# zhanwenchen/pbe

Hardware: AMD Instinct MI355X
Metric: 512x512 images/sec @50 PLMS steps scale=5 (higher is better)
Workload: dtype fp16; 1 GPU; BASELINE configs[1]: batch=4/GPU, 512x512, 50 PLMS steps (51 U-Net calls at batch 8), scale=5, fp16 activations + fp32 accumulate, name-seeded random-init U-Net + VAE + CLIP ViT-L/14 weights; the context-independent prefix of each guidance pair (first ResBlock + first self-attention) is evaluated once; per_gpu_batch=4, global_batch=4, plms_steps=50, parallelism=batch-sharded x1, no per-step collective

## Files before the change

### pbe_amd/csrc/igemm_kernel.h

```cpp
#pragma once
#include <cstddef>
#include <type_traits>
#include <utility>
#include "common.h"
#include "../../include/pbe_hip.h"

struct IGemmP {
    const h16* A; const h16* A2; const h16* W;
    long lda, lda2, ldw;
    long sA, sW;
    int M, N, K, K1;
    int splits;
    int m_fast;
    int tdiv; unsigned mg_tdiv;
    int split_per;
    int sv_ns;
    int sv_gdiv; unsigned mg_sv_gdiv;
    int H, Wd, C1, C2, Ho, Wo, cstride, pad, ups, cb;
    int phase;
    int th;
    int hw; unsigned mg_hw, mg_wo;
    int per_blk; unsigned mg_per_blk, mg_kb;
    int h_hw2, h_hps, h_nsub, h_rows, h_tpi; unsigned mg_h_tpi, mh_hps, mh_hw2; int h_lgw, h_lgimg;
    h16* C;
// ... 130 lines not shown
                    const float v = 8 * c + 4 * q + e < len ? (float)x[4 * q + e] * al : 0.f;
                    word |= mx8_e4m3(v * inv) << (8 * e);
                }
                w[2 * cc + q] = (int)word;
            }
        }
        *reinterpret_cast<i32x4_*>(dst + 16 * hf) = w;
    }
    return se;
}

__device__ __forceinline__ int mx8_range(const IGemmP& p, int n) {
    int r = -1;
    for (int q = 0; q < p.mx_nr; ++q)
        if (p.mx_c0[q] <= n && (r < 0 || p.mx_c0[q] > p.mx_c0[r])) r = q;
    return r;
}

__device__ __forceinline__ void mx8_vt_scale(const IGemmP& p, int r, int b, int c, int tok, int se) {
    const int D = p.mx_D, DV = p.mx_DV;
    const int h = c / D, d = c - h * D;
    unsigned char* sp = p.mx_scale[r] + (((long)b * p.mx_H + h) * (p.mx_N >> 5) + (tok >> 5)) * DV;
    sp[d] = (unsigned char)se;
    if (d == D - 1)
        for (int q = D; q < DV; q += 8) *reinterpret_cast<unsigned long long*>(sp + q) = 0x7f7f7f7f7f7f7f7full;
}

__device__ __forceinline__ void mx8_vt_block(const IGemmP& p, int r, const h16* src, int b, int c, int tok) {
    const int se = mx8_block_lds(src, 32, p.mx_alpha[r], p.mx_data[r] + ((long)b * p.mx_H * p.mx_D + c) * p.mx_N + tok);
    mx8_vt_scale(p, r, b, c, tok, se);
}

__device__ __forceinline__ void mx8_vt_block_pair(const IGemmP& p, int r, const h16* src, int b, int c, int tok, int hf) {
    typedef int i32x4_ __attribute__((ext_vector_type(4)));
    const float al = p.mx_alpha[r];
    const h16x8 x[2] = {*reinterpret_cast<const h16x8*>(src + 16 * hf), *reinterpret_cast<const h16x8*>(src + 16 * hf + 8)};
    float amax = 0.f;
#pragma unroll
    for (int c2 = 0; c2 < 2; ++c2)
#pragma unroll
        for (int e = 0; e < 8; ++e) amax = fmaxf(amax, fabsf((float)x[c2][e] * al));
    amax = fmaxf(amax, __shfl_xor(amax, 32, 64));
    const int se = mx8_scale_exp(amax);
    const float inv = __uint_as_float((unsigned)(254 - se) << 23);
    i32x4_ w;
#pragma unroll
    for (int q = 0; q < 4; ++q) {
        unsigned word = 0;
#pragma unroll
        for (int e = 0; e < 4; ++e) word |= mx8_e4m3((float)x[q >> 1][4 * (q & 1) + e] * al * inv) << (8 * e);
        w[q] = (int)word;
    }
    *reinterpret_cast<i32x4_*>(p.mx_data[r] + ((long)b * p.mx_H * p.mx_D + c) * p.mx_N + tok + 16 * hf) = w;
    if (hf == 0) mx8_vt_scale(p, r, b, c, tok, se);
}

__device__ __forceinline__ void mx8_token_blocks(const IGemmP& p, int r, const h16* st, int ld, int rows, int x0, int cols, int mrow0, int t0, int nt) {
    const int D = p.mx_D, Hh = p.mx_H, Nt = p.mx_N, DP = p.mx_DP;
    const int nbh = (D + 31) >> 5, npb = DP >> 5;
    auto nblk = [&](int x) { const int hh = x / D; return hh * nbh + (x - hh * D + 31) / 32; };
    const int c0 = p.mx_c0[r], rel0 = x0 - c0, rel1 = min(x0 + cols, c0 + Hh * D) - c0;
    if (rel1 <= rel0) return;
    const int b0 = nblk(rel0), cnt = nblk(rel1) - b0;
    const float al = p.mx_alpha[r];
    for (int idx = t0; idx < rows * cnt; idx += nt) {
        const int row = idx / cnt, gb = b0 + (idx - row * cnt);
        const int m = mrow0 + row;
        if (m >= p.M) continue;
        const int h = gb / nbh, j = gb - h * nbh, len = min(32, D - 32 * j);
        unsigned char* dst = p.mx_data[r] + (long)m * Hh * DP + h * DP + 32 * j;
        const int se = mx8_block_lds(st + row * ld + (c0 + h * D + 32 * j - x0), len, al, dst);
        const int b = m / Nt, n = m - b * Nt;
        unsigned char* sp = p.mx_scale[r] + (((long)b * Hh + h) * npb + j) * Nt + n;
        sp[0] = (unsigned char)se;
        if (j == nbh - 1 && npb > nbh) {
            typedef int i32x4_ __attribute__((ext_vector_type(4)));
            *reinterpret_cast<i32x4_*>(dst + 32) = (i32x4_){0, 0, 0, 0};
            *reinterpret_cast<i32x4_*>(dst + 48) = (i32x4_){0, 0, 0, 0};
            sp[Nt] = 127;
        }
    }
}

template <int BM, int BN, int NWM, int NWN, int MODE, int S, int HPA = 0, bool PP = false, bool F8 = false, int EX = 0>
#ifndef PBE_EX_MINWAVES
#define PBE_EX_MINWAVES 2
#endif
__global__ void __launch_bounds__(NWM* NWN * 64, ((EX & 4) != 0 && NWM * NWN == 4 && S == 2) ? PBE_EX_MINWAVES : 1) igemm_kernel(const IGemmP p) {
    constexpr bool EXL = (EX & 1) != 0, EXS = (EX & 2) != 0, EXV = (EX & 4) != 0, EXM = (EX & EX_MX) != 0;
    constexpr int EXF = EX & 7;
    constexpr int NW = NWM * NWN, NT = NW * 64;
    constexpr int D = S - 1;
    constexpr int WM = BM / NWM, WN = BN / NWN, TM = WM / 16, TN = WN / 16;
    constexpr int A_BYTES = BM * 128, W_BYTES = BN * 128, STAGE = A_BYTES + W_BYTES;
    constexpr int PA = BM / 8, PW = BN / 8;
    constexpr int LA = PA / NW, LW = (PW + NW - 1) / NW, LPT = LA + LW;
    constexpr int CLD = BN + 8;
    constexpr int RING = MODE == 2 ? 2 * HPA * 128 + S * W_BYTES : S * STAGE;
    static_assert(S >= 2 && S <= 4 && PA % NW == 0 && BM % 16 == 0 && BN % 16 == 0, "A pieces must divide over the waves (weight pieces may be padded)");
    static_assert(MODE != 2 || (HPA % 8 == 0 && HPA >= BM), "halo image must hold the tile");
    static_assert(EXF == 0 || (MODE == 0 && !F8), "extended epilogue: dense fp16 tiles only");
    static_assert(!EXM || (MODE == 0 && !EXS && (F8 || EXF == (EX_LN | EX_VT))), "MX-fp8 copy-out: the fp8 tiles and the q|k|v^T form");
    extern __shared__ __attribute__((aligned(16))) unsigned char smem[];

    const int tid = threadIdx.x, lane = tid & 63;
    const int wave = __builtin_amdgcn_readfirstlane(tid >> 6);
    const int wm = wave % NWM, wn = wave / NWM;
    PBE_ACC_DECL;
#if PBE_PRIO_MODE == 2
    if (NW == 8 && __builtin_amdgcn_readfirstlane(wave) >= 4) __builtin_amdgcn_s_setprio(1);
#endif
    PBE_STAMP(0);
    PBE_STAMP(7);
    int tile;
    {
        const int nwg = gridDim.x, id = blockIdx.x, q = nwg >> 3, r = nwg & 7, xcd = id & 7;
        tile = (xcd < r ? xcd * (q + 1) : r * (q + 1) + (xcd - r) * q) + (id >> 3);
    }
    const int tq = (int)udiv_mg((unsigned)tile, (unsigned)p.tdiv, p.mg_tdiv), tr = tile - tq * p.tdiv;
    const int tn_i = p.m_fast ? tq : tr, tm_i = p.m_fast ? tr : tq;
    const int m0 = tm_i * BM, n0 = tn_i * BN;
    const long bz = blockIdx.y;
#ifdef PBE_STAMPS
    if (m0 >= 0) PBE_STAMP(14);
#endif

    const int lrow = lane >> 3;
    const int gch = (lane & 7) ^ lrow;
    const h16* zsrc = reinterpret_cast<const h16*>(g_pbe_zero16);

    const h16* a_cur[LA];
    const h16* a_alt[LA];
#pragma unroll
    for (int i = 0; i < LA; ++i) {
        const int m = min(m0 + (wave * LA + i) * 8 + lrow, p.M - 1);
        a_cur[i] = p.A + bz * p.sA + (long)m * p.lda + gch * 8;
        a_alt[i] = p.A2 ? p.A2 + (long)m * p.lda2 + gch * 8 - p.K1 : a_cur[i];
    }
    int* tab = reinterpret_cast<int*>(smem + RING);
    float* svec = reinterpret_cast<float*>(smem + (RING > WM * CLD * 2 ? RING : WM * CLD * 2) + (MODE == 1 ? 9 * BM * 4 : 0));
    const int sv_ns = p.sv_ns;
    if (MODE == 1) {
        const int hw = p.hw, Hv = p.H << p.ups, Wv = p.Wd << p.ups;
        const int py = p.phase ? (int)(blockIdx.y >> 1) : 0, px = p.phase ? (int)(blockIdx.y & 1) : 0;
        for (int row = tid; row < BM; row += NT) {
            const int m = m0 + row;
            const bool rok = m < p.M;
            const int b = (int)udiv_mg((unsigned)m, (unsigned)hw, p.mg_hw), rem = m - b * hw;
            const int oy = (int)udiv_mg((unsigned)rem, (unsigned)p.Wo, p.mg_wo), ox = rem - oy * p.Wo;
            const int iy0 = oy * p.cstride - p.pad, ix0 = ox * p.cstride - p.pad;
            if (p.phase) {
#pragma unroll
                for (int tp = 0; tp < 4; ++tp) {
                    const int iy = oy - 1 + py + (tp >> 1), ix = ox - 1 + px + (tp & 1);
                    const bool ok = rok && (unsigned)iy < (unsigned)p.H && (unsigned)ix < (unsigned)p.Wd;
                    tab[tp * BM + row] = ok ? (b * p.H + iy) * p.Wd + ix : -1;
                }
                continue;
            }
#pragma unroll
            for (int tp = 0; tp < 9; ++tp) {
                const int iy = iy0 + tp / 3, ix = ix0 + tp % 3;
                const bool ok = rok && (unsigned)iy < (unsigned)Hv && (unsigned)ix < (unsigned)Wv;
                tab[tp * BM + row] = ok ? (b * p.H + (iy >> p.ups)) * p.Wd + (ix >> p.ups) : -1;
            }
        }
// ... 541 lines not shown
            const int nl = wn * WN + i * 16 + fq * 4;
            const int n = n0 + nl;
            float ali = al, c1a[4] = {0.f, 0.f, 0.f, 0.f};
            if constexpr (EXV) ali = (p.alpha_cols > 0 && n >= p.alpha_cols) ? 1.f : al;
            if constexpr (EXL) {
                if (EXF != 7 || p.ln_stat) {
                    const f32x4 c1 = *reinterpret_cast<const f32x4*>(lnc + nl);
#pragma unroll
                    for (int r = 0; r < 4; ++r) c1a[r] = ali * c1[r];
                }
            }
            float bn[4] = {0.f, 0.f, 0.f, 0.f};
            if (F) {
                const f32x4 t = *reinterpret_cast<const f32x4*>(svec + nl);
#pragma unroll
                for (int r = 0; r < 4; ++r) bn[r] = t[r];
            } else if (!p.sv_ok && p.bias && !p.bias_row) {
#pragma unroll
                for (int r = 0; r < 4; ++r) bn[r] = (n + r < p.N) ? p.bias[n + r] : 0.f;
            }
#pragma unroll
            for (int j = 0; j < TM; ++j) {
                const int ml = (ONE_PASS ? wm * WM : 0) + j * 16 + fr;
                float v[4];
                float add[4] = {bn[0], bn[1], bn[2], bn[3]};
                if (!F) {
                    const int m = m0 + g * GR + ml;
                    if (p.sv_ok) {
                        const f32x4 t = *reinterpret_cast<const f32x4*>(svec + (sv_ns > 1 ? (g * GR + ml) / p.group_rows : 0) * BN + nl);
#pragma unroll
                        for (int r = 0; r < 4; ++r) add[r] = t[r];
                    } else if (p.rowvec && m < p.M) {
                        const h16* rv = p.rowvec + (long)(m / p.group_rows) * p.ldv + n;
#pragma unroll
                        for (int r = 0; r < 4; ++r)
                            if (n + r < p.N) add[r] = bn[r] + (float)rv[r];
                    }
                }
                if constexpr (F8) {
                    const float sm = sca[g * GR + ml] * al;
                    const f32x4 sn = *reinterpret_cast<const f32x4*>(scw + nl);
#pragma unroll
                    for (int r = 0; r < 4; ++r) v[r] = __builtin_fmaf(acc[i][j][r], sm * sn[r], add[r]);
                } else if constexpr (EXF != 0) {
                    if constexpr (EXL && EXF != 7) {
                        const float ars = ali * ln_rs[j];
#pragma unroll
                        for (int r = 0; r < 4; ++r) v[r] = __builtin_fmaf(acc[i][j][r], ars, __builtin_fmaf(ln_nm[j], c1a[r], add[r]));
                    } else {
                        const float ars = (EXL && p.ln_stat) ? ali * ln_rs[j] : ali, nmj = (EXL && p.ln_stat) ? ln_nm[j] : 0.f;
#pragma unroll
                        for (int r = 0; r < 4; ++r) v[r] = __builtin_fmaf(acc[i][j][r], ars, __builtin_fmaf(nmj, c1a[r], add[r]));
                    }
                    if constexpr (VT) {
#pragma unroll
                        for (int r = 0; r < 4; ++r) sC[(nl + r) * CLDT + ml] = (h16)v[r];
                        continue;
                    }
                } else {
#pragma unroll
                    for (int r = 0; r < 4; ++r) v[r] = __builtin_fmaf(acc[i][j][r], al, add[r]);
                }
                if (!F) {
                    const int m = m0 + g * GR + ml;
                    if (p.bias && p.bias_row) {
                        const float bm = (m < p.M) ? p.bias[m] : 0.f;
#pragma unroll
                        for (int r = 0; r < 4; ++r) v[r] += bm;
                    }
                }
                if (A == PBE_ACT_GEGLU) {
                    h16x2 o2 = {(h16)(v[0] * gelu_erf_f(v[1])), (h16)(v[2] * gelu_erf_f(v[3]))};
                    *reinterpret_cast<h16x2*>(sC + ml * CLD + (nl >> 1)) = o2;
                } else {
                    apply_act4(v, A);
                    h16x4 o;
#pragma unroll
                    for (int r = 0; r < 4; ++r) o[r] = (h16)v[r];
                    *reinterpret_cast<h16x4*>(sC + ml * CLD + nl) = o;
                }
            }
        }
    };
    auto copy_out = [&](int g, auto GG) {
        constexpr bool gg = decltype(GG)::value;
        constexpr int cpr = gg ? CPR / 2 : CPR;
        constexpr int TOT = GR * cpr, IT = (TOT + NT - 1) / NT;
        constexpr int UB = !ONE_PASS ? (IT % 2 == 0 ? 2 : 1) : (IT % 5 == 0 ? 5 : (IT % 4 == 0 ? 4 : (IT % 3 == 0 ? 3 : (IT % 2 == 0 ? 2 : 1))));
        const int Nout = gg ? p.N >> 1 : p.N, nb = gg ? n0 >> 1 : n0;
        if constexpr (EXM && !gg) {
            if (p.mx_crow) {
                constexpr int BPR = BN / 32;
                for (int idx = tid; idx < GR * BPR; idx += NT) {
                    const int row = idx / BPR, cb = idx - row * BPR;
                    const int m = m0 + g * GR + row, n = n0 + cb * 32;
                    if (m >= p.M || n >= p.N) continue;
                    mx8_vt_block(p, 0, sC + row * CLD + cb * 32, (int)bz, m, n);
                }
                return;
            }
            const int r = mx8_range(p, n0);
            if (r < 0) return;
            if (p.mx_layout[r] == PBE_MX8_VT) {
                if constexpr (EXV) {
                    constexpr int BPR = GR / 32;
                    for (int idx = tid; idx < BN * BPR; idx += NT) {
                        const int crow = idx / BPR, tb = idx - crow * BPR;
                        const int m = m0 + tb * 32;
                        if (m >= p.M || n0 + crow >= p.N) continue;
                        const int b = m / p.mx_N;
                        mx8_vt_block(p, r, sC + crow * CLDT + tb * 32, b, n0 - p.mx_c0[r] + crow, m - b * p.mx_N);
                    }
                }
                return;
            }
            mx8_token_blocks(p, r, sC, CLD, GR, n0, BN, m0 + g * GR, tid, NT);
            return;
        }
        if constexpr (EXV && !gg) {
            if (vtile) {
                constexpr int tpr = GR / 8;
                for (int idx = tid; idx < BN * tpr; idx += NT) {
                    const int crow = idx / tpr, tch = idx - crow * tpr;
                    const int m = m0 + tch * 8, c = n0 - p.vt_col0 + crow;
                    if (m >= p.M || n0 + crow >= p.N) continue;
                    const int b = m / p.vt_tok, tok = m - b * p.vt_tok;
                    *reinterpret_cast<h16x8*>(p.vt + (long)b * p.vt_bs + (long)c * p.vt_rs + tok) = *reinterpret_cast<const h16x8*>(sC + crow * CLDT + tch * 8);
                }
                return;
            }
        }
        if constexpr (EXS && !gg) {
            if (p.rstat) {
                constexpr int RPP = NT / 8, CPL = (CPR + 7) / 8, NIT = (GR + RPP - 1) / RPP;
                const int l8 = tid & 7, rr = tid >> 3;
                h16x8 r[NIT][CPL];
                if (Rb) {
#pragma unroll
                    for (int it = 0; it < NIT; ++it) {
                        const int row = it * RPP + rr, m = m0 + g * GR + row;
#pragma unroll
                        for (int c = 0; c < CPL; ++c) {
                            const int ch = l8 + 8 * c, n = n0 + ch * 8;
                            if (row < GR && m < p.M && ch < CPR && n < p.N) r[it][c] = *reinterpret_cast<const h16x8*>(Rb + (long)m * p.ldr + n);
                        }
                    }
                }
#pragma unroll
                for (int it = 0; it < NIT; ++it) {
                    const int row = it * RPP + rr, m = m0 + g * GR + row;
                    const bool rok = row < GR && m < p.M;
                    float s1 = 0.f, s2 = 0.f;
#pragma unroll
                    for (int c = 0; c < CPL; ++c) {
                        const int ch = l8 + 8 * c, n = n0 + ch * 8;
                        if (!(rok && ch < CPR && n < p.N)) continue;
                        h16x8 v = *reinterpret_cast<const h16x8*>(sC + row * CLD + ch * 8);
                        if (Rb) {
#pragma unroll
                            for (int e = 0; e < 8; ++e) v[e] = (h16)((float)v[e] + (float)r[it][c][e]);
                        }
#pragma unroll
                        for (int e = 0; e < 8; ++e) { const float f = (float)v[e]; s1 += f; s2 = __builtin_fmaf(f, f, s2); }
                        *reinterpret_cast<h16x8*>(Cb + (long)m * p.ldc + n) = v;
                    }
#pragma unroll
                    for (int o = 1; o < 8; o <<= 1) { s1 += __shfl_xor(s1, o, 64); s2 += __shfl_xor(s2, o, 64); }
                    if (rok && l8 == 0) *reinterpret_cast<float2*>(p.rstat + 2 * ((long)tn_i * p.rstat_ld + m)) = make_float2(s1, s2);
                }
                return;
            }
        }
        if constexpr (GS_OK && !gg) {
            if (p.gstat) {
                constexpr int RSL = NT / CPR, GB = 4;
                float* red = reinterpret_cast<float*>(smem + GS_OFF);
                const int slot = tid / CPR, ch = tid - slot * CPR, n = n0 + ch * 8;
                float ca[8], cq[8];
#pragma unroll
                for (int e = 0; e < 8; ++e) { ca[e] = 0.f; cq[e] = 0.f; }
                if (slot < RSL && n < p.N) {
                    for (int r0 = slot; r0 < GR; r0 += RSL * GB) {
                        h16x8 v[GB], r[GB];
                        bool ok[GB];
#pragma unroll
                        for (int u = 0; u < GB; ++u) {
                            const int row = r0 + u * RSL, m = m0 + row;
                            ok[u] = row < GR && m < p.M;
                            if (ok[u] && Rb) r[u] = *reinterpret_cast<const h16x8*>(Rb + (long)m * p.ldr + n);
                        }
#pragma unroll
                        for (int u = 0; u < GB; ++u)
                            if (ok[u]) v[u] = *reinterpret_cast<const h16x8*>(sC + (r0 + u * RSL) * CLD + ch * 8);
#pragma unroll
                        for (int u = 0; u < GB; ++u) {
                            if (!ok[u]) continue;
                            if (Rb) {
#pragma unroll
                                for (int e = 0; e < 8; ++e) v[u][e] = (h16)((float)v[u][e] + (float)r[u][e]);
                            }
#pragma unroll
                            for (int e = 0; e < 8; ++e) { const float f = (float)v[u][e]; ca[e] += f; cq[e] = __builtin_fmaf(f, f, cq[e]); }
                            *reinterpret_cast<h16x8*>(Cb + out_row(m0 + r0 + u * RSL) * p.ldc + n) = v[u];
                        }
                    }
                }
                if (slot < RSL) {
#pragma unroll
                    for (int e = 0; e < 8; ++e) *reinterpret_cast<float2*>(red + ((slot * BN) + ch * 8 + e) * 2) = make_float2(ca[e], cq[e]);
                }
                __syncthreads();
                float* col = red + RSL * BN * 2;
                if (tid < BN) {
                    float a = 0.f, q = 0.f;
                    for (int sl = 0; sl < RSL; ++sl) { const float2 t = *reinterpret_cast<const float2*>(red + (sl * BN + tid) * 2); a += t.x; q += t.y; }
                    *reinterpret_cast<float2*>(col + tid * 2) = make_float2(a, q);
                }
                __syncthreads();
                const int cg = p.gs_cg, gl = tid;
                if (gl * cg < BN && n0 + gl * cg < p.N) {
                    float a = 0.f, q = 0.f;
                    for (int c = gl * cg; c < (gl + 1) * cg; ++c) { const float2 t = *reinterpret_cast<const float2*>(col + c * 2); a += t.x; q += t.y; }
                    const int b = m0 / p.gs_hw, blk = (m0 - b * p.gs_hw) / BM, nblk = p.gs_hw / BM;
                    *reinterpret_cast<float2*>(p.gstat + (((long)b * nblk + blk) * p.gs_groups + n0 / cg + gl) * 2) = make_float2(a, q);
                }
                return;
            }
        }
        if (p.vec) {
            for (int it0 = 0; it0 < IT; it0 += UB) {
                h16x8 v[UB], r[UB];
                long go[UB];
                int lo[UB];
#pragma unroll
                for (int u = 0; u < UB; ++u) {
                    const int idx = tid + (it0 + u) * NT;
                    const int row = idx / cpr, ch = idx - row * cpr;
                    const int m = m0 + g * GR + row, n = nb + ch * 8;
                    const bool ok = idx < TOT && m < p.M && n < Nout;
                    go[u] = ok ? out_row(m) * p.ldc + n : -1;
                    lo[u] = row * CLD + ch * 8;
                    if (ok && Rb) r[u] = *reinterpret_cast<const h16x8*>(Rb + (long)m * p.ldr + n);
                }
#pragma unroll
                for (int u = 0; u < UB; ++u)
                    if (go[u] >= 0) v[u] = *reinterpret_cast<const h16x8*>(sC + lo[u]);
#pragma unroll
                for (int u = 0; u < UB; ++u) {
                    if (go[u] < 0) continue;
                    if (Rb) {
#pragma unroll
                        for (int e = 0; e < 8; ++e) v[u][e] = (h16)((float)v[u][e] + (float)r[u][e]);
                    }
                    *reinterpret_cast<h16x8*>(Cb + go[u]) = v[u];
                }
            }
            return;
        }
        for (int idx = tid; idx < TOT; idx += NT) {
            const int row = idx / cpr, ch = idx - row * cpr;
            const int m = m0 + g * GR + row, n = nb + ch * 8;
            if (m >= p.M || n >= Nout) continue;
            const h16x8 v = *reinterpret_cast<const h16x8*>(sC + row * CLD + ch * 8);
#pragma unroll
            for (int e = 0; e < 8; ++e) {
                if (n + e < Nout) {
                    float f = (float)v[e];
                    if (Rb) f += (float)Rb[(long)m * p.ldr + n + e];
                    Cb[out_row(m) * p.ldc + n + e] = (h16)f;
                }
            }
        }
    };
    const bool fast = p.sv_ok && sv_ns == 1 && !(p.bias && p.bias_row);
#pragma unroll 1
    for (int g = 0; g < NG; ++g) {
        __syncthreads();
        if (ONE_PASS || wm == g) {
            auto run = [&](auto FAST) {
                if constexpr (EXV) {
                    if (vtile) { stage(g, FAST, std::integral_constant<int, 0>{}, std::true_type{}); return; }
                }
                if constexpr (ARMS) {
                    switch (p.act) {
                        case 1: stage(g, FAST, std::integral_constant<int, 1>{}, std::false_type{}); break;
                        case 2: stage(g, FAST, std::integral_constant<int, 2>{}, std::false_type{}); break;
                        case 3: stage(g, FAST, std::integral_constant<int, 3>{}, std::false_type{}); break;
                        case PBE_ACT_GEGLU: stage(g, FAST, std::integral_constant<int, PBE_ACT_GEGLU>{}, std::false_type{}); break;
                        default: stage(g, FAST, std::integral_constant<int, 0>{}, std::false_type{}); break;
                    }
                } else {
                    stage(g, FAST, std::integral_constant<int, -1>{}, std::false_type{});
                }
            };
            if (fast) run(std::true_type{});
            else run(std::false_type{});
        }
        __syncthreads();
#ifdef PBE_STAMPS
        if (g == NG - 1) PBE_STAMP(5);
#endif
        if (p.act == PBE_ACT_GEGLU) copy_out(g, std::true_type{});
        else copy_out(g, std::false_type{});
    }
    PBE_STAMP(6);
    PBE_STAMP(8);
}

static __global__ void __launch_bounds__(256) splitk_reduce_kernel(const IGemmP p) {
    const long i = (long)blockIdx.x * 256 + threadIdx.x;
    const int n4 = p.N >> 2;
    if (i >= (long)p.M * n4) return;
    const int m = (int)(i / n4), n = (int)(i - (long)m * n4) * 4;
    float ev[4] = {0.f, 0.f, 0.f, 0.f}, rs[4] = {0.f, 0.f, 0.f, 0.f};
    if (p.bias) {
#pragma unroll
        for (int r = 0; r < 4; ++r) ev[r] = p.bias_row ? p.bias[m] : p.bias[n + r];
    }
    if (p.rowvec) {
        const h16* rv = p.rowvec + (long)(m / p.group_rows) * p.ldv + n;
#pragma unroll
        for (int r = 0; r < 4; ++r) ev[r] += (float)rv[r];
    }
    if (p.resid && p.act != PBE_ACT_GEGLU) {
#pragma unroll
        for (int r = 0; r < 4; ++r) rs[r] = (float)p.resid[(long)m * p.ldr + n + r];
    }
    const float* sl = p.ws + (long)m * p.N + n;
    const long zs = (long)p.M * p.N;
    f32x4 a = {0.f, 0.f, 0.f, 0.f};
    int z = 0;
    for (; z + 4 <= p.splits; z += 4) {
        const f32x4 t0 = *reinterpret_cast<const f32x4*>(sl + (z + 0) * zs), t1 = *reinterpret_cast<const f32x4*>(sl + (z + 1) * zs);
        const f32x4 t2 = *reinterpret_cast<const f32x4*>(sl + (z + 2) * zs), t3 = *reinterpret_cast<const f32x4*>(sl + (z + 3) * zs);
        a += t0; a += t1; a += t2; a += t3;
    }
    for (; z < p.splits; ++z) a += *reinterpret_cast<const f32x4*>(sl + z * zs);
    float v[4];
#pragma unroll
    for (int r = 0; r < 4; ++r) v[r] = a[r] * p.alpha + ev[r];
    if (p.act == PBE_ACT_GEGLU) {
        h16x2 o2 = {(h16)(v[0] * gelu_erf_f(v[1])), (h16)(v[2] * gelu_erf_f(v[3]))};
        *reinterpret_cast<h16x2*>(p.C + (long)m * p.ldc + (n >> 1)) = o2;
        return;
    }
    h16x4 o;
#pragma unroll
    for (int r = 0; r < 4; ++r) {
        const float f = (float)(h16)apply_act(v[r], p.act) + rs[r];
        o[r] = (h16)f;
    }
    *reinterpret_cast<h16x4*>(p.C + (long)m * p.ldc + n) = o;
}

static inline bool al16(const void* p) { return (reinterpret_cast<uintptr_t>(p) & 15) == 0; }
struct Plan { int cfg; int splits; };
enum : unsigned {
    F_DENSE = 1u << 0,
    F_CONV = 1u << 1,
    F_HALO = 1u << 2,
    F_EX = 1u << 3,
    F_F8 = 1u << 4,
    F_ASTAT = 1u << 5,
    F_FORCED = 1u << 6,
};
struct TileCfg { int bm, bn, nwm, nwn, s, slots_per_cu; double eff, eff_shallow; int hpa; unsigned forms; int f8; };
static constexpr TileCfg kTiles[] = {
    {256, 256, 2, 4, 2, 1, 1.00, 0.82, 0, F_DENSE | F_CONV, 3},
    {256, 128, 4, 2, 3, 1, 0.82, 0.72, 0, F_DENSE | F_CONV, 3},
    {128, 256, 2, 4, 3, 1, 0.75, 0.66, 0, F_DENSE | F_CONV, 3},
    {128, 128, 2, 2, 2, 2, 0.88, 1.00, 0, F_DENSE | F_CONV | F_EX | F_F8, 3},
    {128, 64, 2, 2, 2, 3, 0.65, 0.84, 0, F_DENSE | F_CONV | F_EX | F_F8, 4},
    {64, 128, 2, 2, 2, 3, 0.65, 0.85, 0, F_DENSE | F_CONV | F_EX, 6},
    {64, 64, 2, 2, 2, 4, 0.60, 0.80, 0, F_DENSE | F_CONV | F_EX | F_F8, 6},
    {256, 320, 2, 4, 2, 1, 1.05, 0.80, 0, F_DENSE | F_CONV, 8},
    {128, 320, 2, 4, 2, 1, 0.96, 0.95, 0, F_DENSE | F_CONV | F_EX | F_F8, 8},
    {128, 160, 2, 2, 2, 2, 0.90, 0.97, 0, F_DENSE | F_CONV | F_EX | F_F8, 9},
    {256, 160, 4, 2, 3, 1, 1.40, 1.40, 392, F_HALO, 9},
    {128, 160, 4, 2, 3, 1, 1.20, 1.20, 264, F_HALO, 9},
    {128, 320, 2, 4, 2, 1, 1.25, 1.25, 264, F_HALO, 9},
    {256, 128, 4, 2, 3, 1, 1.30, 1.30, 392, F_HALO, 9},
// ... 246 lines not shown
```

### pbe_amd/csrc/norm.hip

```cpp
#include "common.h"
#include "../../include/pbe_hip.h"

#define GN_MAX_C 4096
#define GN_MAX_CHUNKS 256

__device__ __forceinline__ const h16* gn_src(const h16* X, const h16* X2, int C1, int C2, long row, int v) {
    const int c = v * 8;
    return (c < C1) ? X + row * C1 + c : X2 + row * C2 + (c - C1);
}

__global__ void __launch_bounds__(256) gn_stats_kernel(const h16* X, const h16* X2, float* part, int HW, int C1, int C2,
                                                        int groups, int rows_per_block, int TX, int TY) {
    __shared__ float s_sum[GN_MAX_C], s_sq[GN_MAX_C];
    __shared__ float s_pa[256 * 8], s_pq[256 * 8];
    const int C = C1 + C2, C8 = C >> 3, cg = C / groups;
    const int tid = threadIdx.x, tx = tid % TX, ty = tid / TX;
    const int b = blockIdx.y, chunk = blockIdx.x;
    const int r0 = chunk * rows_per_block;
    const int r1 = min(HW, r0 + rows_per_block);
    if (ty < TY) {
        for (int v = tx; v < C8; v += TX) {
            float a[8], q[8];
#pragma unroll
            for (int e = 0; e < 8; ++e) { a[e] = 0.f; q[e] = 0.f; }
            int r = r0 + ty;
            for (; r + 3 * TY < r1; r += 4 * TY) {
                h16x8 x[4];
#pragma unroll
                for (int u = 0; u < 4; ++u) x[u] = *reinterpret_cast<const h16x8*>(gn_src(X, X2, C1, C2, (long)b * HW + r + u * TY, v));
#pragma unroll
                for (int u = 0; u < 4; ++u)
#pragma unroll
                    for (int e = 0; e < 8; ++e) { const float f = (float)x[u][e]; a[e] += f; q[e] += f * f; }
            }
            for (; r < r1; r += TY) {
                const h16x8 x = *reinterpret_cast<const h16x8*>(gn_src(X, X2, C1, C2, (long)b * HW + r, v));
#pragma unroll
                for (int e = 0; e < 8; ++e) { const float f = (float)x[e]; a[e] += f; q[e] += f * f; }
            }
            if (TY == 1) {
#pragma unroll
                for (int e = 0; e < 8; ++e) { s_sum[v * 8 + e] = a[e]; s_sq[v * 8 + e] = q[e]; }
            } else {
#pragma unroll
                for (int e = 0; e < 8; ++e) { s_pa[tid * 8 + e] = a[e]; s_pq[tid * 8 + e] = q[e]; }
            }
        }
    }
    __syncthreads();
    if (TY > 1) {
        for (int c = tid; c < C; c += 256) {
            const int v = c >> 3, e = c & 7;
            float a = 0.f, q = 0.f;
            for (int y = 0; y < TY; ++y) { a += s_pa[(y * TX + v) * 8 + e]; q += s_pq[(y * TX + v) * 8 + e]; }
            s_sum[c] = a; s_sq[c] = q;
        }
        __syncthreads();
    }
    if (tid < groups) {
        float a = 0.f, q = 0.f;
        for (int c = tid * cg; c < (tid + 1) * cg; ++c) { a += s_sum[c]; q += s_sq[c]; }
        float* dst = part + (((long)b * gridDim.x + chunk) * groups + tid) * 2;
        dst[0] = a; dst[1] = q;
    }
}

__global__ void __launch_bounds__(256) gn_apply_kernel(const h16* X, const h16* X2, const float* part, const float* gamma,
                                                        const float* beta, h16* Y, int HW, int C1, int C2, int groups,
                                                        int nchunks, int rows_per_block, int TX, int TY, float eps, int silu) {
    __shared__ float s_mean[64], s_rstd[64];
    __shared__ double s_a[256], s_q[256];
    const int C = C1 + C2, C8 = C >> 3, cg = C / groups;
    const int tid = threadIdx.x, tx = tid % TX, ty = tid / TX;
    const int b = blockIdx.y;
    {
        const int slices = 256 / groups;
        const int g = tid % groups, sl = tid / groups;
        double a = 0.0, q = 0.0;
        if (sl < slices)
            for (int c = sl; c < nchunks; c += slices) {
                const float* src = part + (((long)b * nchunks + c) * groups + g) * 2;
                a += (double)src[0]; q += (double)src[1];
            }
        s_a[tid] = a; s_q[tid] = q;
        __syncthreads();
        if (tid < groups) {
            double ta = 0.0, tq = 0.0;
            for (int s = 0; s < slices; ++s) { ta += s_a[s * groups + tid]; tq += s_q[s * groups + tid]; }
            const double n = (double)HW * cg;
            const double mean = ta / n;
            double var = tq / n - mean * mean;
            if (var < 0.0) var = 0.0;
            s_mean[tid] = (float)mean;
            s_rstd[tid] = (float)(1.0 / sqrt(var + (double)eps));
        }
        __syncthreads();
    }
    const int r0 = blockIdx.x * rows_per_block;
    const int r1 = min(HW, r0 + rows_per_block);
    if (ty >= TY) return;
    for (int v = tx; v < C8; v += TX) {
        float sc[8], sh[8];
#pragma unroll
        for (int e = 0; e < 8; ++e) {
            const int c = v * 8 + e, g = c / cg;
            const float a = s_rstd[g] * gamma[c];
            sc[e] = a; sh[e] = beta[c] - s_mean[g] * a;
        }
        int r = r0 + ty;
        for (; r + 3 * TY < r1; r += 4 * TY) {
            h16x8 x[4];
#pragma unroll
            for (int u = 0; u < 4; ++u) x[u] = *reinterpret_cast<const h16x8*>(gn_src(X, X2, C1, C2, (long)b * HW + r + u * TY, v));
#pragma unroll
            for (int u = 0; u < 4; ++u) {
                h16x8 y;
#pragma unroll
                for (int e = 0; e < 8; ++e) {
                    float f = (float)x[u][e] * sc[e] + sh[e];
                    if (silu) f = silu_f(f);
                    y[e] = (h16)f;
                }
                *reinterpret_cast<h16x8*>(Y + ((long)b * HW + r + u * TY) * C + v * 8) = y;
            }
        }
        for (; r < r1; r += TY) {
            const long row = (long)b * HW + r;
            const h16x8 x = *reinterpret_cast<const h16x8*>(gn_src(X, X2, C1, C2, row, v));
            h16x8 y;
#pragma unroll
            for (int e = 0; e < 8; ++e) {
                float f = (float)x[e] * sc[e] + sh[e];
                if (silu) f = silu_f(f);
                y[e] = (h16)f;
            }
            *reinterpret_cast<h16x8*>(Y + row * C + v * 8) = y;
        }
    }
}

#define GN_SMALL_ROWS 12
__global__ void __launch_bounds__(256) gn_small_kernel(const h16* X, const h16* X2, const float* gamma, const float* beta, h16* Y,
                                                        int HW, int C1, int C2, int groups, float eps, int silu) {
    __shared__ float s_a[4], s_q[4];
    const int C = C1 + C2, cg = C / groups, TX = cg >> 3, TY = 256 / TX;
    const int tid = threadIdx.x, lane = tid & 63, wave = tid >> 6;
    const int tx = tid % TX, ty = tid / TX;
    const int g = blockIdx.x, b = blockIdx.y;
    const int v = (g * cg >> 3) + tx;
    const bool act = ty < TY;
    h16x8 x[GN_SMALL_ROWS];
    float a = 0.f, q = 0.f;
#pragma unroll
    for (int u = 0; u < GN_SMALL_ROWS; ++u) {
        const int r = ty + u * TY;
        if (act && r < HW) {
            x[u] = *reinterpret_cast<const h16x8*>(gn_src(X, X2, C1, C2, (long)b * HW + r, v));
#pragma unroll
            for (int e = 0; e < 8; ++e) { const float f = (float)x[u][e]; a += f; q += f * f; }
        }
    }
    a = wave_sum(a); q = wave_sum(q);
    if (lane == 0) { s_a[wave] = a; s_q[wave] = q; }
    __syncthreads();
    const double n = (double)HW * cg;
    const double mean = ((double)s_a[0] + s_a[1] + s_a[2] + s_a[3]) / n;
    double var = ((double)s_q[0] + s_q[1] + s_q[2] + s_q[3]) / n - mean * mean;
    if (var < 0.0) var = 0.0;
    const float mu = (float)mean, rstd = (float)(1.0 / sqrt(var + (double)eps));
    if (!act) return;
    float sc[8], sh[8];
#pragma unroll
    for (int e = 0; e < 8; ++e) {
        const int c = v * 8 + e;
        sc[e] = rstd * gamma[c];
        sh[e] = beta[c] - mu * sc[e];
    }
#pragma unroll
    for (int u = 0; u < GN_SMALL_ROWS; ++u) {
        const int r = ty + u * TY;
        if (r < HW) {
            h16x8 y;
#pragma unroll
            for (int e = 0; e < 8; ++e) {
                float f = (float)x[u][e] * sc[e] + sh[e];
                if (silu) f = silu_f(f);
                y[e] = (h16)f;
            }
            *reinterpret_cast<h16x8*>(Y + ((long)b * HW + r) * C + v * 8) = y;
        }
    }
}

int g_pbe_gn_rows = 16;
int g_pbe_gn_apply2_rows = 8;
int g_pbe_gn_apply_rows = 4;
static void gn_geometry(int HW, int C, int* nchunks, int* rpb, int* TX, int* TY, int rows_per_thread = 0) {
    const int C8 = C / 8;
    *TX = C8 < 256 ? C8 : 256;
    *TY = 256 / *TX;
    int rows = *TY * (rows_per_thread > 0 ? rows_per_thread : g_pbe_gn_rows);
    if (rows < 32) rows = 32;
    int n = (HW + rows - 1) / rows;
    if (n > GN_MAX_CHUNKS) { n = GN_MAX_CHUNKS; rows = (HW + n - 1) / n; n = (HW + rows - 1) / rows; }
    *nchunks = n; *rpb = rows;
}

extern "C" size_t pbe_groupnorm_workspace_bytes(int32_t B, int32_t HW) {
    (void)HW;
    return (size_t)B * GN_MAX_CHUNKS * 64 * 2 * sizeof(float);
}

extern "C" int pbe_groupnorm_f16(const void* X, const void* X2, const float* gamma, const float* beta, void* Y, int32_t B,
                                 int32_t HW, int32_t C1, int32_t C2, int32_t groups, float eps, int32_t silu, void* workspace,
                                 size_t workspace_bytes, pbe_stream_t stream) {
    const int C = C1 + C2;
    PBE_REQUIRE(X && gamma && beta && Y && workspace, "pbe_groupnorm_f16: null operand");
    PBE_REQUIRE(B > 0 && HW > 0 && C1 > 0 && C2 >= 0, "pbe_groupnorm_f16: bad dims");
    PBE_REQUIRE((C2 == 0) == (X2 == nullptr), "pbe_groupnorm_f16: X2 / C2 mismatch");
    PBE_REQUIRE(C1 % 8 == 0 && C2 % 8 == 0 && C <= GN_MAX_C, "pbe_groupnorm_f16: C1=%d C2=%d must be multiples of 8, total <= %d", C1, C2, GN_MAX_C);
    PBE_REQUIRE(groups > 0 && groups <= 64 && C % groups == 0, "pbe_groupnorm_f16: groups=%d must divide C=%d (<= 64)", groups, C);
    PBE_REQUIRE(B <= 65535, "pbe_groupnorm_f16: batch too large");
    PBE_REQUIRE(workspace_bytes >= pbe_groupnorm_workspace_bytes(B, HW), "pbe_groupnorm_f16: workspace too small");
    hipStream_t s = (hipStream_t)stream;
    const int cg = C / groups;
    if (cg % 8 == 0 && cg / 8 <= 64 && HW <= GN_SMALL_ROWS * (256 / (cg / 8))) {
        pbe_prof_begin(PBE_K_GNORM, s);
        hipLaunchKernelGGL(gn_small_kernel, dim3(groups, B), dim3(256), 0, s, (const h16*)X, (const h16*)X2, gamma, beta, (h16*)Y, HW, C1, C2,
                           groups, eps, silu);
        pbe_prof_end(PBE_K_GNORM, s, 4.0 * B * (double)HW * C);
        PBE_LAUNCH_CHECK("pbe_groupnorm_f16");
        return PBE_OK;
    }
    int nchunks, rpb, TX, TY;
    gn_geometry(HW, C, &nchunks, &rpb, &TX, &TY);
    pbe_prof_begin(PBE_K_GNORM, s);
    hipLaunchKernelGGL(gn_stats_kernel, dim3(nchunks, B), dim3(256), 0, s, (const h16*)X, (const h16*)X2, (float*)workspace, HW, C1, C2,
                       groups, rpb, TX, TY);
    {
        int ac = nchunks, arpb = rpb, aTX = TX, aTY = TY;
        if (g_pbe_gn_apply2_rows > 0) gn_geometry(HW, C, &ac, &arpb, &aTX, &aTY, g_pbe_gn_apply2_rows);
        hipLaunchKernelGGL(gn_apply_kernel, dim3(ac, B), dim3(256), 0, s, (const h16*)X, (const h16*)X2, (const float*)workspace, gamma,
                           beta, (h16*)Y, HW, C1, C2, groups, nchunks, arpb, aTX, aTY, eps, silu);
    }
    pbe_prof_end(PBE_K_GNORM, s, 6.0 * B * (double)HW * C);
    PBE_LAUNCH_CHECK("pbe_groupnorm_f16");
    return PBE_OK;
}

extern "C" int pbe_groupnorm_apply_f16(const void* X, const float* partials, int32_t blocks, const float* gamma, const float* beta, void* Y,
                                       int32_t B, int32_t HW, int32_t C, int32_t groups, float eps, int32_t silu, pbe_stream_t stream) {
    PBE_REQUIRE(X && partials && gamma && beta && Y, "pbe_groupnorm_apply_f16: null operand");
    PBE_REQUIRE(B > 0 && B <= 65535 && HW > 0 && C > 0 && C % 8 == 0 && C <= GN_MAX_C && blocks > 0, "pbe_groupnorm_apply_f16: bad dims");
    PBE_REQUIRE(groups > 0 && groups <= 64 && C % groups == 0, "pbe_groupnorm_apply_f16: groups=%d must divide C=%d (<= 64)", groups, C);
    hipStream_t s = (hipStream_t)stream;
    int nchunks, rpb, TX, TY;
    gn_geometry(HW, C, &nchunks, &rpb, &TX, &TY, g_pbe_gn_apply_rows);
    pbe_prof_begin(PBE_K_GNORM, s);
    hipLaunchKernelGGL(gn_apply_kernel, dim3(nchunks, B), dim3(256), 0, s, (const h16*)X, (const h16*)nullptr, partials, gamma, beta, (h16*)Y, HW, C, 0,
// ... 238 lines not shown
```

Before: 8.150 images/sec.

## Prefetch residual tiles in GEMM epilogue and hoist GroupNorm loads before statistics

The igemm epilogue now loads residual (Rb) vectors into registers ahead of use. For some tile configurations it issues them before the main epilogue barrier, and it double-buffers them across copy-out batches in the vec, rstat and gstat paths. When pipelined, the epilogue barriers become an explicit lgkmcnt wait plus s_barrier. The GroupNorm apply kernel prefetches its first four rows and its gamma/beta before computing the statistics, and gn_small loads gamma/beta before its reduction. All of this aims to hide global-memory latency behind LDS and reduction work, at the cost of more registers and possible occupancy loss.

```diff
diff --git a/pbe_amd/csrc/igemm_kernel.h b/pbe_amd/csrc/igemm_kernel.h
--- a/pbe_amd/csrc/igemm_kernel.h
+++ b/pbe_amd/csrc/igemm_kernel.h
@@ -236,6 +236,22 @@
     }
 }
 
+constexpr int igemm_copy_ub(bool one_pass, int it) {
+    return !one_pass ? (it % 2 == 0 ? 2 : 1) : (it % 5 == 0 ? 5 : (it % 4 == 0 ? 4 : (it % 3 == 0 ? 3 : (it % 2 == 0 ? 2 : 1))));
+}
+
+constexpr int igemm_resid_prefetch(int bm, int bn, int nw, int s, int mode, bool f8, int ex, bool one_pass) {
+    if (!one_pass) return -1;
+#ifdef PBE_RESID_PF
+    return PBE_RESID_PF;
+#endif
+    if (bm == 128 && bn == 160 && nw == 4 && s == 2 && mode == 0) return f8 ? 1 : ((ex & 7) == 1 ? 0 : 2);
+    return 2;
+}
+constexpr int igemm_rs_early(int bm, int bn, int nw, int s, int ex, int nit) {
+    return (bm == 128 && bn == 160 && nw == 4 && s == 2 && (ex & 7) == 2) ? 2 : nit;
+}
+
 template <int BM, int BN, int NWM, int NWN, int MODE, int S, int HPA = 0, bool PP = false, bool F8 = false, int EX = 0>
 #ifndef PBE_EX_MINWAVES
 #define PBE_EX_MINWAVES 2
@@ -943,11 +959,76 @@
             }
         }
     };
+    constexpr int RS_RPP = NT / 8, RS_CPL = (CPR + 7) / 8, RS_NIT = (GR + RS_RPP - 1) / RS_RPP;
+    constexpr int GS_RSL = NT / CPR, GS_GB = 4, GS_NB = (GR + GS_RSL * GS_GB - 1) / (GS_RSL * GS_GB);
+    constexpr int UB_N = igemm_copy_ub(ONE_PASS, (GR * CPR + NT - 1) / NT), UB_G = igemm_copy_ub(ONE_PASS, (GR * (CPR / 2) + NT - 1) / NT);
+    constexpr int RQ_V = UB_N > UB_G ? UB_N : UB_G, RQ_S = EXS ? RS_NIT * RS_CPL : 0, RQ_GS = GS_OK ? GS_GB : 0;
+    constexpr int RQN = RQ_V > RQ_S ? (RQ_V > RQ_GS ? RQ_V : RQ_GS) : (RQ_S > RQ_GS ? RQ_S : RQ_GS);
+    constexpr int PF = igemm_resid_prefetch(BM, BN, NW, S, MODE, F8, EX, ONE_PASS);
+    constexpr bool PIPE = PF >= 0;
+    constexpr int RS_E = PF == 2 ? igemm_rs_early(BM, BN, NW, S, EX, RS_NIT) : RS_NIT;
+    h16x8 rq[RQN];
+    auto ld_vec = [&](int g, int it0, auto GG, h16x8* r, int tid) {
+        constexpr bool gg = decltype(GG)::value;
+        constexpr int cpr = gg ? CPR / 2 : CPR, TOT = GR * cpr, UB = gg ? UB_G : UB_N;
+        const int Nout = gg ? p.N >> 1 : p.N, nb = gg ? n0 >> 1 : n0;
+#pragma unroll
+        for (int u = 0; u < UB; ++u) {
+            const int idx = tid + (it0 + u) * NT;
+            const int row = idx / cpr, ch = idx - row * cpr;
+            const int m = m0 + g * GR + row, n = nb + ch * 8;
+            h16x8 t = r[u];
+            if (idx < TOT && m < p.M && n < Nout) t = *reinterpret_cast<const h16x8*>(Rb + (long)m * p.ldr + n);
+            r[u] = t;
+        }
+    };
+    auto ld_gs = [&](int r0, h16x8* r, int tid) {
+        const int slot = tid / CPR, n = n0 + (tid - slot * CPR) * 8;
+        if (!(slot < GS_RSL && n < p.N)) return;
+#pragma unroll
+        for (int u = 0; u < GS_GB; ++u) {
+            const int row = r0 + u * GS_RSL, m = m0 + row;
+            h16x8 t = r[u];
+            if (row < GR && m < p.M) t = *reinterpret_cast<const h16x8*>(Rb + (long)m * p.ldr + n);
+            r[u] = t;
+        }
+    };
+    auto ld_rs = [&](int g, h16x8* r, int tid, auto IT0, auto IT1) {
+        const int l8 = tid & 7, rr = tid >> 3;
+#pragma unroll
+        for (int it = decltype(IT0)::value; it < decltype(IT1)::value; ++it) {
+            const int row = it * RS_RPP + rr, m = m0 + g * GR + row;
+#pragma unroll
+            for (int c = 0; c < RS_CPL; ++c) {
+                const int ch = l8 + 8 * c, n = n0 + ch * 8;
+                h16x8 t = r[it * RS_CPL + c];
+                if (row < GR && m < p.M && ch < CPR && n < p.N) t = *reinterpret_cast<const h16x8*>(Rb + (long)m * p.ldr + n);
+                r[it * RS_CPL + c] = t;
+            }
+        }
+    };
+    auto fetch_first = [&](int g, h16x8* r) {
+        int t = tid;
+        asm volatile("" : "+v"(t));
+        if (!Rb || p.act == PBE_ACT_GEGLU || !(p.vec || (EXS && p.rstat) || (GS_OK && p.gstat))) return;
+        if constexpr (EXM) return;
+        if constexpr (EXV) {
+            if (vtile) return;
+        }
+        if constexpr (EXS) {
+            if (p.rstat) { ld_rs(g, r, t, std::integral_constant<int, 0>{}, std::integral_constant<int, RS_E>{}); return; }
+        }
+        if constexpr (GS_OK) {
+            if (p.gstat) { ld_gs(t / CPR, r, t); return; }
+        }
+        ld_vec(g, 0, std::false_type{}, r, t);
+    };
     auto copy_out = [&](int g, auto GG) {
         constexpr bool gg = decltype(GG)::value;
         constexpr int cpr = gg ? CPR / 2 : CPR;
         constexpr int TOT = GR * cpr, IT = (TOT + NT - 1) / NT;
-        constexpr int UB = !ONE_PASS ? (IT % 2 == 0 ? 2 : 1) : (IT % 5 == 0 ? 5 : (IT % 4 == 0 ? 4 : (IT % 3 == 0 ? 3 : (IT % 2 == 0 ? 2 : 1))));
+        constexpr int UB = gg ? UB_G : UB_N;
+        constexpr bool HAVE = PF > 0 && !gg;
         const int Nout = gg ? p.N >> 1 : p.N, nb = gg ? n0 >> 1 : n0;
         if constexpr (EXM && !gg) {
             if (p.mx_crow) {
@@ -995,18 +1076,9 @@
             if (p.rstat) {
                 constexpr int RPP = NT / 8, CPL = (CPR + 7) / 8, NIT = (GR + RPP - 1) / RPP;
                 const int l8 = tid & 7, rr = tid >> 3;
-                h16x8 r[NIT][CPL];
-                if (Rb) {
-#pragma unroll
-                    for (int it = 0; it < NIT; ++it) {
-                        const int row = it * RPP + rr, m = m0 + g * GR + row;
-#pragma unroll
-                        for (int c = 0; c < CPL; ++c) {
-                            const int ch = l8 + 8 * c, n = n0 + ch * 8;
-                            if (row < GR && m < p.M && ch < CPR && n < p.N) r[it][c] = *reinterpret_cast<const h16x8*>(Rb + (long)m * p.ldr + n);
-                        }
-                    }
-                }
+                static_assert(RPP == RS_RPP && CPL == RS_CPL && NIT == RS_NIT, "ld_rs walks the same chunks");
+                h16x8* r = rq;
+                if (Rb) ld_rs(g, r, tid, std::integral_constant<int, HAVE ? RS_E : 0>{}, std::integral_constant<int, RS_NIT>{});
 #pragma unroll
                 for (int it = 0; it < NIT; ++it) {
                     const int row = it * RPP + rr, m = m0 + g * GR + row;
@@ -1019,7 +1091,7 @@
                         h16x8 v = *reinterpret_cast<const h16x8*>(sC + row * CLD + ch * 8);
                         if (Rb) {
 #pragma unroll
-                            for (int e = 0; e < 8; ++e) v[e] = (h16)((float)v[e] + (float)r[it][c][e]);
+                            for (int e = 0; e < 8; ++e) v[e] = (h16)((float)v[e] + (float)r[it * CPL + c][e]);
                         }
 #pragma unroll
                         for (int e = 0; e < 8; ++e) { const float f = (float)v[e]; s1 += f; s2 = __builtin_fmaf(f, f, s2); }
@@ -1040,16 +1112,18 @@
                 float ca[8], cq[8];
 #pragma unroll
                 for (int e = 0; e < 8; ++e) { ca[e] = 0.f; cq[e] = 0.f; }
+                static_assert(RSL == GS_RSL && GB == GS_GB, "ld_gs walks the same rows");
                 if (slot < RSL && n < p.N) {
-                    for (int r0 = slot; r0 < GR; r0 += RSL * GB) {
-                        h16x8 v[GB], r[GB];
+                    h16x8 rb[GB];
+                    auto batch = [&](int r0, h16x8* r, h16x8* rnext) {
+                        h16x8 v[GB];
                         bool ok[GB];
 #pragma unroll
                         for (int u = 0; u < GB; ++u) {
                             const int row = r0 + u * RSL, m = m0 + row;
                             ok[u] = row < GR && m < p.M;
-                            if (ok[u] && Rb) r[u] = *reinterpret_cast<const h16x8*>(Rb + (long)m * p.ldr + n);
                         }
+                        if (Rb && r0 + RSL * GB < GR) ld_gs(r0 + RSL * GB, rnext, tid);
 #pragma unroll
                         for (int u = 0; u < GB; ++u)
                             if (ok[u]) v[u] = *reinterpret_cast<const h16x8*>(sC + (r0 + u * RSL) * CLD + ch * 8);
@@ -1064,6 +1138,12 @@
                             for (int e = 0; e < 8; ++e) { const float f = (float)v[u][e]; ca[e] += f; cq[e] = __builtin_fmaf(f, f, cq[e]); }
                             *reinterpret_cast<h16x8*>(Cb + out_row(m0 + r0 + u * RSL) * p.ldc + n) = v[u];
                         }
+                    };
+                    if (!HAVE && Rb) ld_gs(slot, rq, tid);
+#pragma unroll
+                    for (int k = 0; k < GS_NB; ++k) {
+                        if (k & 1) batch(slot + k * RSL * GB, rb, rq);
+                        else batch(slot + k * RSL * GB, rq, rb);
                     }
                 }
                 if (slot < RSL) {
@@ -1089,31 +1169,68 @@
             }
         }
         if (p.vec) {
-            for (int it0 = 0; it0 < IT; it0 += UB) {
-                h16x8 v[UB], r[UB];
-                long go[UB];
-                int lo[UB];
-#pragma unroll
-                for (int u = 0; u < UB; ++u) {
-                    const int idx = tid + (it0 + u) * NT;
-                    const int row = idx / cpr, ch = idx - row * cpr;
-                    const int m = m0 + g * GR + row, n = nb + ch * 8;
-                    const bool ok = idx < TOT && m < p.M && n < Nout;
-                    go[u] = ok ? out_row(m) * p.ldc + n : -1;
-                    lo[u] = row * CLD + ch * 8;
-                    if (ok && Rb) r[u] = *reinterpret_cast<const h16x8*>(Rb + (long)m * p.ldr + n);
-                }
-#pragma unroll
-                for (int u = 0; u < UB; ++u)
-                    if (go[u] >= 0) v[u] = *reinterpret_cast<const h16x8*>(sC + lo[u]);
-#pragma unroll
-                for (int u = 0; u < UB; ++u) {
-                    if (go[u] < 0) continue;
-                    if (Rb) {
-#pragma unroll
-                        for (int e = 0; e < 8; ++e) v[u][e] = (h16)((float)v[u][e] + (float)r[u][e]);
-                    }
-                    *reinterpret_cast<h16x8*>(Cb + go[u]) = v[u];
+            if constexpr (PIPE) {
+                h16x8 rb[UB];
+                auto batch = [&](int it0, h16x8* r, h16x8* rnext) {
+                    h16x8 v[UB];
+                    long go[UB];
+                    int lo[UB];
+#pragma unroll
+                    for (int u = 0; u < UB; ++u) {
+                        const int idx = tid + (it0 + u) * NT;
+                        const int row = idx / cpr, ch = idx - row * cpr;
+                        const int m = m0 + g * GR + row, n = nb + ch * 8;
+                        const bool ok = idx < TOT && m < p.M && n < Nout;
+                        go[u] = ok ? out_row(m) * p.ldc + n : -1;
+                        lo[u] = row * CLD + ch * 8;
+                    }
+                    if (Rb && it0 + UB < IT) ld_vec(g, it0 + UB, GG, rnext, tid);
+#pragma unroll
+                    for (int u = 0; u < UB; ++u)
+                        if (go[u] >= 0) v[u] = *reinterpret_cast<const h16x8*>(sC + lo[u]);
+#pragma unroll
+                    for (int u = 0; u < UB; ++u) {
+                        if (go[u] < 0) continue;
+                        if (Rb) {
+#pragma unroll
+                            for (int e = 0; e < 8; ++e) v[u][e] = (h16)((float)v[u][e] + (float)r[u][e]);
+                        }
+                        *reinterpret_cast<h16x8*>(Cb + go[u]) = v[u];
+                    }
+                };
+                if (!HAVE && Rb) ld_vec(g, 0, GG, rq, tid);
+#pragma unroll
+                for (int k = 0; k < IT / UB; ++k) {
+                    if (k & 1) batch(k * UB, rb, rq);
+                    else batch(k * UB, rq, rb);
+                }
+            } else {
+                for (int it0 = 0; it0 < IT; it0 += UB) {
+                    h16x8 v[UB], r[UB];
+                    long go[UB];
+                    int lo[UB];
+#pragma unroll
+                    for (int u = 0; u < UB; ++u) {
+                        const int idx = tid + (it0 + u) * NT;
+                        const int row = idx / cpr, ch = idx - row * cpr;
+                        const int m = m0 + g * GR + row, n = nb + ch * 8;
+                        const bool ok = idx < TOT && m < p.M && n < Nout;
+                        go[u] = ok ? out_row(m) * p.ldc + n : -1;
+                        lo[u] = row * CLD + ch * 8;
+                        if (ok && Rb) r[u] = *reinterpret_cast<const h16x8*>(Rb + (long)m * p.ldr + n);
+                    }
+#pragma unroll
+                    for (int u = 0; u < UB; ++u)
+                        if (go[u] >= 0) v[u] = *reinterpret_cast<const h16x8*>(sC + lo[u]);
+#pragma unroll
+                    for (int u = 0; u < UB; ++u) {
+                        if (go[u] < 0) continue;
+                        if (Rb) {
+#pragma unroll
+                            for (int e = 0; e < 8; ++e) v[u][e] = (h16)((float)v[u][e] + (float)r[u][e]);
+                        }
+                        *reinterpret_cast<h16x8*>(Cb + go[u]) = v[u];
+                    }
                 }
             }
             return;
@@ -1134,9 +1251,19 @@
         }
     };
     const bool fast = p.sv_ok && sv_ns == 1 && !(p.bias && p.bias_row);
+    auto lds_barrier = [] {
+        if constexpr (PIPE) {
+            asm volatile("s_waitcnt lgkmcnt(0)" ::: "memory");
+            __builtin_amdgcn_s_barrier();
+        } else {
+            __syncthreads();
+        }
+    };
+    if constexpr (PIPE) wait_vmcnt<0>();
+    if constexpr (PF == 2) fetch_first(0, rq);
 #pragma unroll 1
     for (int g = 0; g < NG; ++g) {
-        __syncthreads();
+        lds_barrier();
         if (ONE_PASS || wm == g) {
             auto run = [&](auto FAST) {
                 if constexpr (EXV) {
@@ -1157,7 +1284,8 @@
             if (fast) run(std::true_type{});
             else run(std::false_type{});
         }
-        __syncthreads();
+        if constexpr (PF == 1) fetch_first(0, rq);
+        lds_barrier();
 #ifdef PBE_STAMPS
         if (g == NG - 1) PBE_STAMP(5);
 #endif
diff --git a/pbe_amd/csrc/norm.hip b/pbe_amd/csrc/norm.hip
--- a/pbe_amd/csrc/norm.hip
+++ b/pbe_amd/csrc/norm.hip
@@ -73,6 +73,17 @@
     const int C = C1 + C2, C8 = C >> 3, cg = C / groups;
     const int tid = threadIdx.x, tx = tid % TX, ty = tid / TX;
     const int b = blockIdx.y;
+    const int r0 = blockIdx.x * rows_per_block;
+    const int r1 = min(HW, r0 + rows_per_block);
+    h16x8 xp[4];
+    float gp[8], bp[8];
+    if (ty < TY && tx < C8) {
+#pragma unroll
+        for (int u = 0; u < 4; ++u)
+            if (r0 + ty + u * TY < r1) xp[u] = *reinterpret_cast<const h16x8*>(gn_src(X, X2, C1, C2, (long)b * HW + r0 + ty + u * TY, tx));
+#pragma unroll
+        for (int e = 0; e < 8; ++e) { gp[e] = gamma[tx * 8 + e]; bp[e] = beta[tx * 8 + e]; }
+    }
     {
         const int slices = 256 / groups;
         const int g = tid % groups, sl = tid / groups;
@@ -96,18 +107,8 @@
         }
         __syncthreads();
     }
-    const int r0 = blockIdx.x * rows_per_block;
-    const int r1 = min(HW, r0 + rows_per_block);
     if (ty >= TY) return;
-    for (int v = tx; v < C8; v += TX) {
-        float sc[8], sh[8];
-#pragma unroll
-        for (int e = 0; e < 8; ++e) {
-            const int c = v * 8 + e, g = c / cg;
-            const float a = s_rstd[g] * gamma[c];
-            sc[e] = a; sh[e] = beta[c] - s_mean[g] * a;
-        }
-        int r = r0 + ty;
+    auto stream = [&](int v, const float* sc, const float* sh, int r) {
         for (; r + 3 * TY < r1; r += 4 * TY) {
             h16x8 x[4];
 #pragma unroll
@@ -136,6 +137,39 @@
             }
             *reinterpret_cast<h16x8*>(Y + row * C + v * 8) = y;
         }
+    };
+    if (tx < C8) {
+        float sc[8], sh[8];
+#pragma unroll
+        for (int e = 0; e < 8; ++e) {
+            const int c = tx * 8 + e, g = c / cg;
+            const float a = s_rstd[g] * gp[e];
+            sc[e] = a; sh[e] = bp[e] - s_mean[g] * a;
+        }
+        const int r = r0 + ty;
+#pragma unroll
+        for (int u = 0; u < 4; ++u) {
+            if (r + u * TY >= r1) continue;
+            h16x8 y;
+#pragma unroll
+            for (int e = 0; e < 8; ++e) {
+                float f = (float)xp[u][e] * sc[e] + sh[e];
+                if (silu) f = silu_f(f);
+                y[e] = (h16)f;
+            }
+            *reinterpret_cast<h16x8*>(Y + ((long)b * HW + r + u * TY) * C + tx * 8) = y;
+        }
+        stream(tx, sc, sh, r + 4 * TY);
+    }
+    for (int v = tx + TX; v < C8; v += TX) {
+        float sc[8], sh[8];
+#pragma unroll
+        for (int e = 0; e < 8; ++e) {
+            const int c = v * 8 + e, g = c / cg;
+            const float a = s_rstd[g] * gamma[c];
+            sc[e] = a; sh[e] = beta[c] - s_mean[g] * a;
+        }
+        stream(v, sc, sh, r0 + ty);
     }
 }
 
@@ -160,6 +194,11 @@
             for (int e = 0; e < 8; ++e) { const float f = (float)x[u][e]; a += f; q += f * f; }
         }
     }
+    float gv[8], bv[8];
+    if (act) {
+#pragma unroll
+        for (int e = 0; e < 8; ++e) { gv[e] = gamma[v * 8 + e]; bv[e] = beta[v * 8 + e]; }
+    }
     a = wave_sum(a); q = wave_sum(q);
     if (lane == 0) { s_a[wave] = a; s_q[wave] = q; }
     __syncthreads();
@@ -172,9 +211,8 @@
     float sc[8], sh[8];
 #pragma unroll
     for (int e = 0; e < 8; ++e) {
-        const int c = v * 8 + e;
-        sc[e] = rstd * gamma[c];
-        sh[e] = beta[c] - mu * sc[e];
+        sc[e] = rstd * gv[e];
+        sh[e] = bv[e] - mu * sc[e];
     }
 #pragma unroll
     for (int u = 0; u < GN_SMALL_ROWS; ++u) {
```

Result: no change. 8.177 images/sec, median of 6 (+0.3%).
